# duanyiqun/DiffusionDepth

Hardware: NVIDIA H100
Metric: depth maps/sec @ KITTI 352x1216, Swin-L, 20 DDIM steps (higher is better)
Workload: dtype f32 (fp32-grade products on wgmma: 3-pass fp16 split, fp32 accumulate)

## Files before the change

### diffusiondepth_b200/csrc/conv_halo.cuh

```cuda
#pragma once
#include "conv_common.cuh"

namespace dd {

constexpr int HALO_TH = 16;
constexpr int HALO_TW = 8;

template <int CIN, int COUT, int BK>
struct HaloCfg {
  static_assert(BK == 16 || BK == 32, "bad K chunk");
  static_assert((CIN % BK == 0 || CIN < BK) && CIN % 16 == 0, "bad K chunk");
  static constexpr int KC = (CIN + BK - 1) / BK;
  static constexpr int KSTEPS = (CIN < BK ? CIN : BK) / 16;
  static constexpr int ROW_BYTES = BK * 2;
  static constexpr int STRIP_ROWS = (HALO_TH + 2) * HALO_TW;
  static constexpr int STRIP_BYTES = STRIP_ROWS * ROW_BYTES;
  static constexpr int STRIP_PAD = (STRIP_BYTES + 1023) / 1024 * 1024;
  static constexpr int DX_STRIDE = 2 * STRIP_PAD;
  static constexpr int A_SLOT = 3 * DX_STRIDE;
  static constexpr int A_SLOTS = 2;
  static constexpr int B_TILE = COUT * ROW_BYTES;
  static constexpr int B_TILE_PAD = (B_TILE + 1023) / 1024 * 1024;
  static constexpr int B_SLOT = 2 * B_TILE_PAD;
  static constexpr int NWG = COUT > 128 ? 2 : 1;
  static constexpr int NW = COUT / NWG;
  static constexpr int THREADS = 128 * (1 + NWG);
  static constexpr int CH = NWG > 1 ? 16 : (NW < 32 ? NW : 32);
  static constexpr int LD = CH + 1;
  static constexpr int STAGE_BYTES = NWG * 128 * LD * 4;
  static constexpr int CTRL_BYTES = 1024;
  static constexpr int BUDGET = 227 * 1024 - 1024 - CTRL_BYTES - STAGE_BYTES - A_SLOTS * A_SLOT;
  static constexpr int B_SLOTS_RAW = BUDGET / B_SLOT;
  static constexpr bool B_RESIDENT = (9 * KC * B_SLOT <= 40 * 1024) && (9 * KC <= B_SLOTS_RAW);
  static constexpr int B_SLOTS = B_RESIDENT ? 9 * KC : (B_SLOTS_RAW > 8 ? 8 : B_SLOTS_RAW);
  static_assert(B_SLOTS >= 2, "B ring too small");
  static_assert(NWG == 1 || B_SLOTS >= 3, "256-wide layers: the producer must be able to run two taps ahead");
  static constexpr int SMEM_BYTES = A_SLOTS * A_SLOT + B_SLOTS * B_SLOT + 1024 + CTRL_BYTES + STAGE_BYTES;
  static_assert(SMEM_BYTES <= 232448, "exceeds the 227 KB dynamic shared memory limit");
  static constexpr int A_TX = 6 * STRIP_BYTES;
  static constexpr int B_TX = 2 * B_TILE;
  static constexpr int GROUP_CH = COUT / 4;
  static constexpr int GPW = NW >= GROUP_CH ? NW / GROUP_CH : 1;
  static_assert(NW % GROUP_CH == 0, "a warpgroup's columns cover whole GroupNorm groups");
};

template <int CIN, int COUT, int BK, int EPI>
__global__ void __launch_bounds__((HaloCfg<CIN, COUT, BK>::THREADS), 1)
conv3x3_halo_kernel(const __grid_constant__ CUtensorMap tmA_hi, const __grid_constant__ CUtensorMap tmA_lo,
                    const __grid_constant__ CUtensorMap tmB_hi, const __grid_constant__ CUtensorMap tmB_lo,
                    const ConvArgs p) {
  using C = HaloCfg<CIN, COUT, BK>;
  constexpr int NW = C::NW;
  extern __shared__ uint8_t smem_raw[];
  uint8_t* smem = reinterpret_cast<uint8_t*>((reinterpret_cast<uintptr_t>(smem_raw) + 1023) & ~uintptr_t(1023));
  uint8_t* a_ring = smem;
  uint8_t* b_ring = smem + C::A_SLOTS * C::A_SLOT;
  uint8_t* ctrl = b_ring + C::B_SLOTS * C::B_SLOT;
  uint64_t* a_full = reinterpret_cast<uint64_t*>(ctrl);
  uint64_t* a_empty = a_full + C::A_SLOTS;
  uint64_t* b_full = a_empty + C::A_SLOTS;
  uint64_t* b_empty = b_full + C::B_SLOTS;
  double* red = reinterpret_cast<double*>(b_empty + C::B_SLOTS);
  float* stage = reinterpret_cast<float*>(ctrl + C::CTRL_BYTES);

  const int warp = threadIdx.x >> 5;
  const int lane = threadIdx.x & 31;

  if (threadIdx.x == 0) {
    tma_prefetch_desc(&tmA_hi);
    tma_prefetch_desc(&tmA_lo);
    tma_prefetch_desc(&tmB_hi);
    tma_prefetch_desc(&tmB_lo);
    for (int s = 0; s < C::A_SLOTS; ++s) {
      mbar_init(&a_full[s], 1);
      mbar_init(&a_empty[s], C::NWG);
    }
    for (int s = 0; s < C::B_SLOTS; ++s) {
      mbar_init(&b_full[s], 1);
      mbar_init(&b_empty[s], C::NWG);
    }
    fence_barrier_init();
  }
  __syncthreads();

  if (warp < 4) {
    if constexpr (C::NWG > 1) setmaxnreg_dec<40>();
    if (warp == 0) {
      const bool leader = elect_one();
      int sa = 0;
      uint32_t pa = 0;
      for (int tile = blockIdx.x; tile < p.num_tiles; tile += gridDim.x) {
        const int tx = tile % p.tiles_x, ty = (tile / p.tiles_x) % p.tiles_y, img = tile / (p.tiles_x * p.tiles_y);
        const int x0 = tx * HALO_TW, y0 = ty * HALO_TH;
        for (int kc = 0; kc < C::KC; ++kc) {
          mbar_wait(&a_empty[sa], pa ^ 1);
          uint8_t* s = a_ring + sa * C::A_SLOT;
          if (leader) {
            mbar_arrive_expect_tx(&a_full[sa], C::A_TX);
#pragma unroll
            for (int dx = 0; dx < 3; ++dx) {
              tma_load_4d(s + (2 * dx) * C::STRIP_PAD, &tmA_hi, &a_full[sa], kc * BK, x0 + dx - 1, y0 - 1, img);
              tma_load_4d(s + (2 * dx + 1) * C::STRIP_PAD, &tmA_lo, &a_full[sa], kc * BK, x0 + dx - 1, y0 - 1, img);
            }
          }
          __syncwarp();
          if (++sa == C::A_SLOTS) {
            sa = 0;
            pa ^= 1;
          }
        }
      }
    } else if (warp == 1) {
      const bool leader = elect_one();
      int sb = 0;
      uint32_t pb = 0;
      for (int tile = blockIdx.x; tile < p.num_tiles; tile += gridDim.x) {
        if (C::B_RESIDENT && tile != static_cast<int>(blockIdx.x)) break;
        for (int kc = 0; kc < C::KC; ++kc) {
          for (int tap = 0; tap < 9; ++tap) {
            mbar_wait(&b_empty[sb], pb ^ 1);
            uint8_t* s = b_ring + sb * C::B_SLOT;
            if (leader) {
              mbar_arrive_expect_tx(&b_full[sb], C::B_TX);
              tma_load_3d(s, &tmB_hi, &b_full[sb], kc * BK, 0, tap);
              tma_load_3d(s + C::B_TILE_PAD, &tmB_lo, &b_full[sb], kc * BK, 0, tap);
            }
            __syncwarp();
            if (++sb == C::B_SLOTS) {
              sb = 0;
              pb ^= 1;
            }
          }
        }
      }
    }
  } else {
    if constexpr (C::NWG > 1) setmaxnreg_inc<232>();
    const int wg = (warp >> 2) - 1;
    const int t = threadIdx.x & 127;
    const int q = t >> 5;
    const bool signal = (t == 0);
    float* S = stage + wg * 128 * C::LD;
    const int m = t;
    const int r = m >> 3, c = m & 7;
    const uint32_t b_off = static_cast<uint32_t>(wg * NW);
    int sa = 0, sb = 0, par = 0;
    uint32_t pa = 0, pb = 0;
    float acc[2][NW / 2];

    for (int tile = blockIdx.x; tile < p.num_tiles; tile += gridDim.x) {
      int prev_b = -1, prev_a = -1;
      auto retire_prev = [&]() {
        mbar_arrive_if(&b_empty[prev_b < 0 ? 0 : prev_b], signal && prev_b >= 0);
        mbar_arrive_if(&a_empty[prev_a < 0 ? 0 : prev_a], signal && prev_a >= 0);
        prev_b = prev_a = -1;
      };
      {
        for (int kc = 0; kc < C::KC; ++kc) {
          mbar_wait(&a_full[sa], pa);
          const uint32_t a_base = smem_u32(a_ring + sa * C::A_SLOT);
          for (int tap = 0; tap < 9; ++tap) {
            const int dy = tap / 3, dx = tap % 3;
            mbar_wait(&b_full[sb], C::B_RESIDENT ? 0u : pb);
            const uint32_t sa_hi = a_base + dx * C::DX_STRIDE + dy * HALO_TW * C::ROW_BYTES;
            const uint32_t sa_lo = sa_hi + C::STRIP_PAD;
            const uint32_t sb_hi = smem_u32(b_ring + sb * C::B_SLOT) + b_off * C::ROW_BYTES;
            const uint32_t sb_lo = sb_hi + C::B_TILE_PAD;
            wgmma_fence();
#pragma unroll
            for (int h = 0; h < 2; ++h) {
              const uint32_t ho = static_cast<uint32_t>(h * 64 * C::ROW_BYTES);
#pragma unroll
              for (int k = 0; k < C::KSTEPS; ++k) {
                const uint64_t a_hi = wgmma_desc(sa_hi + ho + k * 32, C::ROW_BYTES);
                const uint64_t a_lo = wgmma_desc(sa_lo + ho + k * 32, C::ROW_BYTES);
                const uint64_t b_hi = wgmma_desc(sb_hi + k * 32, C::ROW_BYTES);
                const uint64_t b_lo = wgmma_desc(sb_lo + k * 32, C::ROW_BYTES);
                wgmma_f16<NW>(acc[h], a_lo, b_hi, (kc | tap | k) != 0 ? 1u : 0u);
                wgmma_f16<NW>(acc[h], a_hi, b_lo, 1u);
                wgmma_f16<NW>(acc[h], a_hi, b_hi, 1u);
              }
            }
            wgmma_commit();
            wgmma_wait<1>();
            retire_prev();
            if (!C::B_RESIDENT) prev_b = sb;
            if (tap == 8) prev_a = sa;
            if (++sb == C::B_SLOTS) {
              sb = 0;
              pb ^= 1;
            }
          }
          if (++sa == C::A_SLOTS) {
            sa = 0;
            pa ^= 1;
          }
        }
      }
      wgmma_wait<0>();
      wgmma_fence_regs(acc[0]);
      wgmma_fence_regs(acc[1]);
      retire_prev();

      const int tx = tile % p.tiles_x, ty = (tile / p.tiles_x) % p.tiles_y, img = tile / (p.tiles_x * p.tiles_y);
      const int x = tx * HALO_TW + c, y = ty * HALO_TH + r;
      const bool valid = (x < p.W) && (y < p.H);
      const size_t pix = (static_cast<size_t>(img) * p.H + y) * p.W + x;
      const uint32_t vmask = __ballot_sync(0xffffffffu, valid);
      const uint32_t row_off = static_cast<uint32_t>(pix * COUT);
      float tk[C::GPW], tsum[C::GPW], tsq[C::GPW];
#pragma unroll
      for (int g = 0; g < C::GPW; ++g) tk[g] = tsum[g] = tsq[g] = 0.f;
      bool overflow = false;
#pragma unroll
      for (int cj = 0; cj < NW / C::CH; ++cj) {
        const int ch0 = wg * NW + cj * C::CH;
        named_bar_sync(2 + wg, 128);
        stage_acc_cols<NW, C::CH, C::LD>(acc[0], S, 0, cj * C::CH / 8);
        stage_acc_cols<NW, C::CH, C::LD>(acc[1], S, 64, cj * C::CH / 8);
        named_bar_sync(2 + wg, 128);
        float v[C::CH];
#pragma unroll
        for (int j = 0; j < C::CH; ++j) v[j] = fmaf(S[m * C::LD + j], p.acc_scale, __ldg(p.bias + ch0 + j));
        if constexpr (EPI == EPI_F32_STATS) {
          if (valid) {
#pragma unroll
            for (int j = 0; j < C::CH; ++j) {
              const int g = (cj * C::CH + j) / C::GROUP_CH;
              if ((cj * C::CH + j) % C::GROUP_CH == 0) tk[g] = v[j];
              const float d = v[j] - tk[g];
              tsum[g] += d;
              tsq[g] = fmaf(d, d, tsq[g]);
            }
          }
        }
        if constexpr (EPI == EPI_F32_STATS || EPI == EPI_F32) {
#pragma unroll
          for (int j = 0; j < C::CH; ++j) S[m * C::LD + j] = v[j];
          __syncwarp();
          if constexpr (C::CH == 32) {
#pragma unroll 8
            for (int rw = 0; rw < 32; ++rw) {
              const uint32_t o = __shfl_sync(0xffffffffu, row_off, rw) + ch0 + lane;
              if ((vmask >> rw) & 1u) p.y32[o] = S[(q * 32 + rw) * C::LD + lane];
            }
          } else {
            constexpr int RPI = 32 / C::CH;
            const int hsel = lane / C::CH, cl = lane % C::CH;
#pragma unroll 8
            for (int i = 0; i < 32 / RPI; ++i) {
              const int rw = RPI * i + hsel;
              const uint32_t o = __shfl_sync(0xffffffffu, row_off, rw) + ch0 + cl;
              if ((vmask >> rw) & 1u) p.y32[o] = S[(q * 32 + rw) * C::LD + cl];
            }
          }
        } else if (valid) {
          {
            __align__(16) __half hi[C::CH];
            __align__(16) __half lo[C::CH];
#pragma unroll
            for (int j = 0; j < C::CH; ++j) {
              const float s = v[j] * p.split_scale;
              overflow |= (fabsf(s) > 60000.f);
              hi[j] = __float2half_rn(s);
              lo[j] = __float2half_rn(s - __half2float(hi[j]));
            }
            uint4* dh = reinterpret_cast<uint4*>(p.out_hi + pix * COUT + ch0);
            uint4* dl = reinterpret_cast<uint4*>(p.out_lo + pix * COUT + ch0);
#pragma unroll
            for (int j = 0; j < C::CH / 8; ++j) {
              dh[j] = reinterpret_cast<const uint4*>(hi)[j];
              dl[j] = reinterpret_cast<const uint4*>(lo)[j];
            }
          }
        }
      }

      if constexpr (EPI == EPI_F32_STATS) {
        const int cw = wg * 4 + q;
#pragma unroll
        for (int k = 0; k < C::GPW; ++k) {
          const double n = valid ? C::GROUP_CH : 0, kk = tk[k], ds = tsum[k];
          double s = fma(n, kk, ds), s2 = fma(n * kk, kk, fma(2.0 * kk, ds, static_cast<double>(tsq[k])));
#pragma unroll
          for (int o = 16; o > 0; o >>= 1) {
            s += __shfl_xor_sync(0xffffffffu, s, o);
            s2 += __shfl_xor_sync(0xffffffffu, s2, o);
          }
          if (lane == 0) {
            red[((par * 4 * C::NWG + cw) * C::GPW + k) * 2 + 0] = s;
            red[((par * 4 * C::NWG + cw) * C::GPW + k) * 2 + 1] = s2;
          }
        }
        named_bar_sync(1, 128 * C::NWG);
        const int e = threadIdx.x - 128;
        if (e < 8) {
          const int g = e >> 1, which = e & 1;
          const int w0 = C::NWG > 1 ? (g / C::GPW) * 4 : 0, k = C::NWG > 1 ? g % C::GPW : g;
          double tt = 0.0;
#pragma unroll
          for (int w = 0; w < 4 * C::NWG; ++w)
            if (C::NWG == 1 || (w >= w0 && w < w0 + 4)) tt += red[((par * 4 * C::NWG + w) * C::GPW + k) * 2 + which];
          p.stats_partial[(static_cast<size_t>(tile) * 4 + g) * 2 + which] = tt;
        }
        par ^= 1;
      }
      if constexpr (EPI == EPI_SPLIT) {
        if (overflow) atomicOr(p.status, 1);
      }
    }
  }
}

}
```

### diffusiondepth_b200/csrc/engine.cu

```cuda
#include <cuda.h>
#include <cuda_runtime.h>
#include <math.h>
#include <stdio.h>
#include <stdlib.h>
#include <string.h>

#include <algorithm>
#include <map>
#include <string>
#include <vector>

#include "../../include/dd_engine.h"
#include "kernels.cuh"
#include "convgen.cuh"
#include "conv_halo.cuh"
#include "pred_fold.cuh"
#include "swin.cuh"
#include "mpvit.cuh"
#include "backward.cuh"
#include "codec_train.cuh"
#include "producer_train.cuh"

namespace {

// ... 65 lines not shown

int encode_map(CUtensorMap* m, const char* what, cuuint32_t rank, const __half* base, const cuuint64_t* dims,
               const cuuint64_t* strides, const cuuint32_t* box, const cuuint32_t* estr, CUtensorMapSwizzle swizzle,
               CUtensorMapL2promotion l2) {
  const CUresult r = g_encode(m, CU_TENSOR_MAP_DATA_TYPE_FLOAT16, rank, const_cast<__half*>(base), dims, strides, box, estr,
                              CU_TENSOR_MAP_INTERLEAVE_NONE, swizzle, l2, CU_TENSOR_MAP_FLOAT_OOB_FILL_NONE);
  if (r != CUDA_SUCCESS)
    return fail(DD_ERR_CUDA, std::string("cuTensorMapEncodeTiled(") + what + ") failed: " + std::to_string((int)r));
  return DD_OK;
}

int make_nhwc_map(CUtensorMap* m, const char* what, const __half* base, int B, int H, int W, int C, int box_c, int box_w,
                  int box_h, CUtensorMapSwizzle swizzle, int stride = 1, int ld = 0) {
  const cuuint64_t L = ld > 0 ? ld : C;
  const cuuint64_t dims[4] = {(cuuint64_t)C, (cuuint64_t)W, (cuuint64_t)H, (cuuint64_t)B};
  const cuuint64_t strides[3] = {L * 2, (cuuint64_t)W * L * 2, (cuuint64_t)H * W * L * 2};
  const cuuint32_t box[4] = {(cuuint32_t)box_c, (cuuint32_t)box_w, (cuuint32_t)box_h, 1};
  const cuuint32_t estr[4] = {1, (cuuint32_t)stride, (cuuint32_t)stride, 1};
  return encode_map(m, what, 4, base, dims, strides, box, estr, swizzle, CU_TENSOR_MAP_L2_PROMOTION_L2_128B);
}
int make_act_map(CUtensorMap* m, const __half* base, int B, int H, int W, int C, int bk, int stride = 1, int ld = 0) {
  return make_nhwc_map(m, "activation", base, B, H, W, C, bk, dd::TILE_W * stride, dd::TILE_H * stride, swizzle_for(bk),
                       stride, ld);
}
int make_patch_map(CUtensorMap* m, const __half* base, int B, int H, int W) {
  const cuuint64_t px = 256 * 2;
  const cuuint64_t dims[5] = {8, (cuuint64_t)H, (cuuint64_t)W, 32, (cuuint64_t)B};
  const cuuint64_t strides[4] = {(cuuint64_t)W * px, px, 16, (cuuint64_t)H * W * px};
  const cuuint32_t box[5] = {8, dd::F5::PH, dd::F5::PW, 2, 1};
  const cuuint32_t estr[5] = {1, 1, 1, 1, 1};
  return encode_map(m, "patch", 5, base, dims, strides, box, estr, CU_TENSOR_MAP_SWIZZLE_NONE,
                    CU_TENSOR_MAP_L2_PROMOTION_L2_128B);
}
int make_weight_map(CUtensorMap* m, const __half* base, int cout, int cin, int taps, int box_k, int rows, int ld = 0) {
  const cuuint64_t L = ld > 0 ? ld : cin;
  const cuuint64_t dims[3] = {(cuuint64_t)cin, (cuuint64_t)cout, (cuuint64_t)taps};
  const cuuint64_t strides[2] = {L * 2, (cuuint64_t)cout * L * 2};
  const cuuint32_t box[3] = {(cuuint32_t)box_k, (cuuint32_t)rows, 1};
  const cuuint32_t estr[3] = {1, 1, 1};
  return encode_map(m, "weight", 3, base, dims, strides, box, estr, swizzle_for(box_k), CU_TENSOR_MAP_L2_PROMOTION_L2_256B);
}

struct ShapeInfo {
  int cin, cout;
};
constexpr ShapeInfo kShapes[5] = {{16, 64}, {64, 256}, {256, 256}, {256, 64}, {64, 16}};
int shape_id(int cin, int cout) {
  for (int i = 0; i < 5; ++i)
    if (kShapes[i].cin == cin && kShapes[i].cout == cout) return i;
  return -1;
}

constexpr int kHaloBK[5] = {16, 32, 32, 32, 32};

template <int CIN, int COUT, int BK, int EPI>
void conv3x3_kernel(bool simt, const dd::SimtArgs& sa, const CUtensorMap* m, const dd::ConvArgs& a, int sm_count,
                    cudaStream_t st) {
  if (simt) {
    constexpr int CO_T = COUT < 64 ? COUT : 64;
    dd::conv3x3_simt_kernel<CIN, COUT, EPI><<<dim3(a.num_tiles, COUT / CO_T), 256, 0, st>>>(sa);
  } else {
    using C = dd::HaloCfg<CIN, COUT, BK>;
    const int grid = a.num_tiles < sm_count ? a.num_tiles : sm_count;
    dd::conv3x3_halo_kernel<CIN, COUT, BK, EPI><<<grid, C::THREADS, C::SMEM_BYTES, st>>>(m[0], m[1], m[2], m[3], a);
  }
}
template <int CIN, int COUT, int BK>
void conv3x3_epi(int epi, bool simt, const dd::SimtArgs& sa, const CUtensorMap* m, const dd::ConvArgs& a, int sm_count,
                 cudaStream_t st) {
  if (epi == dd::EPI_F32_STATS) conv3x3_kernel<CIN, COUT, BK, dd::EPI_F32_STATS>(simt, sa, m, a, sm_count, st);
  else if (epi == dd::EPI_SPLIT) conv3x3_kernel<CIN, COUT, BK, dd::EPI_SPLIT>(simt, sa, m, a, sm_count, st);
  else conv3x3_kernel<CIN, COUT, BK, dd::EPI_F32>(simt, sa, m, a, sm_count, st);
}

int launch_conv3x3(int sid, int epi, bool simt, dd::ConvArgs& a, const __half* in_hi, const __half* in_lo,
                   float in_scale, const float* w_simt, const CUtensorMap& w_hi, const CUtensorMap& w_lo, int sm_count,
                   cudaStream_t st) {
  const int tw = simt ? dd::TILE_W : dd::HALO_TW, th = simt ? dd::TILE_H : dd::HALO_TH;
  a.tiles_x = (a.W + tw - 1) / tw;
  a.tiles_y = (a.H + th - 1) / th;
  a.num_tiles = a.tiles_x * a.tiles_y * a.B;
  CUtensorMap m[4] = {{}, {}, w_hi, w_lo};
  dd::SimtArgs sa{};
  if (simt) {
    sa.in_hi = in_hi;
    sa.in_lo = in_lo;
    sa.in_inv_scale = 1.f / in_scale;
    sa.w = w_simt;
    sa.c = a;
  } else {
    const int cin = kShapes[sid].cin, bk = kHaloBK[sid];
    int rc;
    if ((rc = make_nhwc_map(&m[0], "strip", in_hi, a.B, a.H, a.W, cin, bk, dd::HALO_TW, dd::HALO_TH + 2, swizzle_for(bk))))
      return rc;
    if ((rc = make_nhwc_map(&m[1], "strip", in_lo, a.B, a.H, a.W, cin, bk, dd::HALO_TW, dd::HALO_TH + 2, swizzle_for(bk))))
      return rc;
  }
  switch (sid) {
    case 0: conv3x3_epi<16, 64, kHaloBK[0]>(epi, simt, sa, m, a, sm_count, st); break;
    case 1: conv3x3_epi<64, 256, kHaloBK[1]>(epi, simt, sa, m, a, sm_count, st); break;
    case 2: conv3x3_epi<256, 256, kHaloBK[2]>(epi, simt, sa, m, a, sm_count, st); break;
    case 3: conv3x3_epi<256, 64, kHaloBK[3]>(epi, simt, sa, m, a, sm_count, st); break;
    case 4: conv3x3_epi<64, 16, kHaloBK[4]>(epi, simt, sa, m, a, sm_count, st); break;
    default: return fail(DD_ERR_UNSUPPORTED, "unsupported conv shape");
  }
  return DD_OK;
}

template <int CIN, int COUT, int BK>
cudaError_t configure_halo_all_epi() {
  using C = dd::HaloCfg<CIN, COUT, BK>;
  cudaError_t e;
  if ((e = cudaFuncSetAttribute(dd::conv3x3_halo_kernel<CIN, COUT, BK, dd::EPI_F32_STATS>,
                                cudaFuncAttributeMaxDynamicSharedMemorySize, C::SMEM_BYTES)) != cudaSuccess) return e;
  if ((e = cudaFuncSetAttribute(dd::conv3x3_halo_kernel<CIN, COUT, BK, dd::EPI_SPLIT>,
                                cudaFuncAttributeMaxDynamicSharedMemorySize, C::SMEM_BYTES)) != cudaSuccess) return e;
  return cudaFuncSetAttribute(dd::conv3x3_halo_kernel<CIN, COUT, BK, dd::EPI_F32>,
                              cudaFuncAttributeMaxDynamicSharedMemorySize, C::SMEM_BYTES);
}
template <int MCO, int NCI>
cudaError_t configure_wgm() {
  return cudaFuncSetAttribute(dd::wgrad_wgmma_kernel<MCO, NCI>, cudaFuncAttributeMaxDynamicSharedMemorySize,
                              dd::WgmCfg<MCO, NCI>::SMEM_BYTES);
}
template <int NT>
cudaError_t configure_gen() {
  return cudaFuncSetAttribute(dd::convgen_wgmma_kernel<NT>, cudaFuncAttributeMaxDynamicSharedMemorySize,
                              dd::GenCfg<NT>::SMEM_BYTES);
}
cudaError_t configure_all_kernels() {
  cudaError_t e;
  if ((e = cudaFuncSetAttribute(dd::window_attention_wgmma_kernel, cudaFuncAttributeMaxDynamicSharedMemorySize,
                                dd::WAU_SMEM)) != cudaSuccess) return e;
  if ((e = cudaFuncSetAttribute(dd::decoder_kernel, cudaFuncAttributeMaxDynamicSharedMemorySize, dd::DEC_SMEM)) != cudaSuccess)
    return e;
  if ((e = configure_halo_all_epi<16, 64, 16>()) != cudaSuccess) return e;
  if ((e = configure_halo_all_epi<64, 256, 32>()) != cudaSuccess) return e;
  if ((e = configure_halo_all_epi<256, 256, 32>()) != cudaSuccess) return e;
  if ((e = configure_halo_all_epi<256, 64, 32>()) != cudaSuccess) return e;
  if ((e = configure_halo_all_epi<64, 16, 32>()) != cudaSuccess) return e;
  if ((e = cudaFuncSetAttribute(dd::conv5x5_fold_kernel, cudaFuncAttributeMaxDynamicSharedMemorySize,
                                dd::F5::SMEM_BYTES)) != cudaSuccess) return e;
  if ((e = cudaFuncSetAttribute(dd::ring_fix_kernel, cudaFuncAttributeMaxDynamicSharedMemorySize, dd::RING_SMEM)) !=
      cudaSuccess) return e;
  if ((e = configure_wgm<128, 128>()) != cudaSuccess) return e;
  if ((e = configure_wgm<128, 64>()) != cudaSuccess) return e;
  if ((e = configure_wgm<64, 128>()) != cudaSuccess) return e;
  if ((e = configure_gen<256>()) != cudaSuccess) return e;
  if ((e = configure_gen<192>()) != cudaSuccess) return e;
  if ((e = configure_gen<128>()) != cudaSuccess) return e;
  return configure_gen<64>();
}

struct ConvLayer {
  int sid = -1;
  __half* w_hi = nullptr;
  __half* w_lo = nullptr;
  float* w_simt = nullptr;
  float* bias = nullptr;
  float wscale = 1.f;
  CUtensorMap mh_hi, mh_lo;
};

struct PackStage {
  float amax[16];
  float dec_wt[16 * 16 * 16], dec_bt[16], dec_g[16], dec_be[16], dec_mu[16], dec_var[16], dec_wc[16 * 9], dec_bc[1];
  float enc_w1[144], enc_bn1[4][16], enc_w2[2304], enc_bn2[4][16];
  float wt_f[4 * 4 * 16 * 16], bt_f[16], wc_f[9 * 16], wu[4 * 4 * 16 * 16], bn[3 * 16];
  float f1[144], t1[16], f2[2304], t2[16];
  float e1u[144], e2u[2304], enc_gb[4][16];
  float enc_bn[2][3][16];
};

struct Raw {
  const float* ptr;
  std::vector<int64_t> shape;
};

struct GenLayer {
  int cin = 0, cout = 0, taps = 1, nt = 256, relu = 1, shuffle = 0;
  int stride = 1, add_first = 0;
  __half* w_hi = nullptr;
  __half* w_lo = nullptr;
  float* shift = nullptr;
  float wscale = 1.f;
  CUtensorMap mb_hi, mb_lo;
  bool alt = false;
  CUtensorMap mb_hi_alt, mb_lo_alt;
  float* zero_shift = nullptr;
  int bn = -1;
};

constexpr int kGenSplitIters = 110;
// ... 845 lines not shown
int poll_status(dd_engine* h, cudaStream_t st) {
  CUDA_TRY(cudaMemcpyAsync(h->status_host, h->status, 4, cudaMemcpyDeviceToHost, st));
  CUDA_TRY(cudaStreamSynchronize(st));
  if (*h->status_host & 1)
    return fail(DD_ERR_RANGE, "an activation exceeded the operand split's range (16 |v| > 6e4)");
  return DD_OK;
}

int finish_forward(dd_engine* h, cudaStream_t st) {
  return (h->cfg.flags & DD_FLAG_CHECK_RANGE) ? poll_status(h, st) : DD_OK;
}

void invalidate_pack(dd_engine* h) {
  h->weights_ready = h->packed = false;
  h->ws = nullptr;
  drop_graphs(h);
}

int check_status_word(const int* status, cudaStream_t st, const char* what) {
  int flag = 0;
  CUDA_TRY(cudaMemcpyAsync(&flag, status, 4, cudaMemcpyDeviceToHost, st));
  CUDA_TRY(cudaStreamSynchronize(st));
  if (flag) return fail(DD_ERR_RANGE, std::string("non-finite or out-of-range value in ") + what);
  return DD_OK;
}

const Raw* find(dd_engine* e, const std::string& k) {
  auto it = e->raw.find(k);
  return it == e->raw.end() ? nullptr : &it->second;
}

int dev_alloc(std::vector<void*>& owned, void** p, size_t bytes) {
  cudaError_t err = cudaMalloc(p, bytes);
  if (err != cudaSuccess) return fail(DD_ERR_CUDA, std::string("cudaMalloc: ") + cudaGetErrorString(err));
  owned.push_back(*p);
  return DD_OK;
}
int dev_alloc(dd_engine* e, void** p, size_t bytes) { return dev_alloc(e->owned, p, bytes); }

template <typename T>
int dev_array(dd_engine* e, T** p, size_t elems) {
  return dev_alloc(e->owned, reinterpret_cast<void**>(p), elems * sizeof(T));
}

int alloc_layer(dd_engine* e, ConvLayer& L, int cout, int cin) {
  L.sid = shape_id(cin, cout);
  if (L.sid < 0) return fail(DD_ERR_UNSUPPORTED, "unsupported conv shape");
  const size_t n = static_cast<size_t>(cout) * cin * 9;
  int rc;
  if ((rc = dev_array(e, &L.w_hi, n))) return rc;
  if ((rc = dev_array(e, &L.w_lo, n))) return rc;
  if ((rc = dev_array(e, &L.w_simt, n))) return rc;
  if ((rc = dev_array(e, &L.bias, cout))) return rc;
  if ((rc = make_weight_map(&L.mh_hi, L.w_hi, cout, cin, 9, kHaloBK[L.sid], cout))) return rc;
  return make_weight_map(&L.mh_lo, L.w_lo, cout, cin, 9, kHaloBK[L.sid], cout);
}

constexpr float kProdScale = 16.f;

void bn_fold_host(const float* const* bn, int ch, float* scale, float* shift) {
  for (int c = 0; c < ch; ++c) {
    const double sc = static_cast<double>(bn[0][c]) / sqrt(static_cast<double>(bn[3][c]) + 1e-5);
    scale[c] = static_cast<float>(sc);
    shift[c] = static_cast<float>(static_cast<double>(bn[1][c]) - static_cast<double>(bn[2][c]) * sc);
  }
}
int bn_fold(const float* const* bn, int ch, std::vector<float>& scale, std::vector<float>& shift, cudaStream_t st) {
  std::vector<float> v[4];
  for (int i = 0; i < 4; ++i) {
    v[i].resize(ch);
    CUDA_TRY(cudaMemcpyAsync(v[i].data(), bn[i], ch * 4, cudaMemcpyDeviceToHost, st));
  }
  CUDA_TRY(cudaStreamSynchronize(st));
  scale.resize(ch);
  shift.resize(ch);
  const float* host[4] = {v[0].data(), v[1].data(), v[2].data(), v[3].data()};
  bn_fold_host(host, ch, scale.data(), shift.data());
  return DD_OK;
}
int find_bn(dd_engine* e, const std::string& prefix, const float** bn) {
  const char* parts[4] = {".weight", ".bias", ".running_mean", ".running_var"};
  for (int i = 0; i < 4; ++i) {
    const Raw* r = find(e, prefix + parts[i]);
    if (!r) return fail(DD_ERR_INVALID, "missing weights: " + prefix + parts[i]);
    bn[i] = r->ptr;
  }
  return DD_OK;
}
int copy_param(dd_engine* e, const std::string& key, size_t n, float** out, cudaStream_t st) {
  const Raw* r = find(e, key);
  if (!r) return fail(DD_ERR_INVALID, "missing weights: " + key);
  size_t have = 1;
  for (int64_t d : r->shape) have *= static_cast<size_t>(d);
  if (have != n) return fail(DD_ERR_INVALID, "weight shape mismatch: " + key);
  int rc;
  if ((rc = dev_alloc(e, reinterpret_cast<void**>(out), n * 4))) return rc;
  CUDA_TRY(cudaMemcpyAsync(*out, r->ptr, n * 4, cudaMemcpyDeviceToDevice, st));
  return DD_OK;
}

const char* const kGnKey[4] = {"model.noise_embedding.1", "model.noise_embedding.4", "model.pred.1", "model.pred.4"};
constexpr int kGnCh[4] = {64, 256, 64, 16};
const std::string kDecPrefix = "depth_transform.conv_inv_transform.";
const std::string kEncPrefix = "depth_transform.conv_transform.";
struct CodecKey {
  const char* leaf;
  size_t host_off;
  std::vector<int64_t> shape;
// ... 2292 lines not shown

int dd_poll_status(dd_handle h, void* cuda_stream) {
  if (!h) return fail(DD_ERR_INVALID, "null handle");
  if (!h->status) return DD_OK;
  CUDA_TRY(cudaSetDevice(h->cfg.device));
  return poll_status(h, static_cast<cudaStream_t>(cuda_stream));
}

size_t dd_conv3x3_workspace_bytes(int32_t batch, int32_t cin, int32_t cout, int32_t height, int32_t width) {
  Conv3x3Ws v;
  return conv3x3_layout(nullptr, batch, cin, cout, height, width, v);
}

int dd_conv3x3(dd_handle h, const float* x, const float* w, const float* b, float* y, int32_t batch, int32_t cin,
               int32_t cout, int32_t height, int32_t width, void* workspace, size_t workspace_bytes, void* cuda_stream) {
  if (!h || !x || !w || !b || !y) return fail(DD_ERR_INVALID, "null argument");
  const int sid = shape_id(cin, cout);
  if (sid < 0) return fail(DD_ERR_UNSUPPORTED, "conv shape not on the DiffusionDepth hot path");
  if (workspace_bytes < dd_conv3x3_workspace_bytes(batch, cin, cout, height, width) ||
      (reinterpret_cast<uintptr_t>(workspace) & 1023))
    return fail(DD_ERR_INVALID, "conv workspace too small or misaligned");
  cudaStream_t st = static_cast<cudaStream_t>(cuda_stream);
  CUDA_TRY(cudaSetDevice(h->cfg.device));
  const size_t BP = static_cast<size_t>(batch) * height * width;
  const size_t nw = static_cast<size_t>(cin) * cout * 9;
  Conv3x3Ws v;
  conv3x3_layout(workspace, batch, cin, cout, height, width, v);
  CUDA_TRY(cudaMemsetAsync(v.status, 0, 64, st));
  int rc;
  if ((rc = transpose_in(x, v.xn, batch, cin, height * width, st))) return rc;
  float* amax_dev = reinterpret_cast<float*>(v.status) + 8;
  float sx, sw;
  if ((rc = split_scale_of(v.xn, std::min<size_t>(BP * cin, 1u << 30), amax_dev, st, &sx))) return rc;
  if ((rc = split_scale_of(w, nw, amax_dev, st, &sw))) return rc;
  dd::split_planes_kernel<<<132 * 8, 256, 0, st>>>(v.xn, v.x.hi, v.x.lo, BP * cin / 4, sx, v.status);
  if ((rc = check_launch("split_planes"))) return rc;
  dd::pack_conv_weight_kernel<<<128, 256, 0, st>>>(w, v.w.hi, v.w.lo, v.wsimt, cout, cin, sw);
  if ((rc = check_launch("pack_conv_weight"))) return rc;
  dd::ConvArgs a;
  a.B = batch;
  a.H = height;
  a.W = width;
  a.bias = b;
  a.acc_scale = 1.f / (sx * sw);
  a.y32 = v.yn;
  a.stats_partial = nullptr;
  a.out_hi = nullptr;
  a.out_lo = nullptr;
  a.split_scale = 1.f;
  a.status = v.status;
  const bool simt = (h->cfg.flags & DD_FLAG_SIMT_CONV) != 0;
  CUtensorMap mb_hi{}, mb_lo{};
  if (!simt) {
    if ((rc = make_weight_map(&mb_hi, v.w.hi, cout, cin, 9, kHaloBK[sid], cout))) return rc;
    if ((rc = make_weight_map(&mb_lo, v.w.lo, cout, cin, 9, kHaloBK[sid], cout))) return rc;
  }
  if ((rc = launch_conv3x3(sid, dd::EPI_F32, simt, a, v.x.hi, v.x.lo, sx, v.wsimt, mb_hi, mb_lo, h->sm_count, st)))
    return rc;
  if ((rc = check_launch("conv3x3"))) return rc;
  return transpose_out(v.yn, y, batch, cout, height * width, st);
}

size_t dd_conv3x3_wgrad_workspace_bytes(int32_t batch, int32_t cin, int32_t cout, int32_t height, int32_t width) {
  WgradWs v;
  return wgrad_layout(nullptr, batch, cin, cout, height, width, v);
}

int dd_conv3x3_wgrad(dd_handle h, const float* x, const float* dy, float* dw, float* db, int32_t batch, int32_t cin,
                     int32_t cout, int32_t height, int32_t width, void* workspace, size_t workspace_bytes,
                     void* cuda_stream) {
  if (!h || !x || !dy || !dw || !db) return fail(DD_ERR_INVALID, "null argument");
  if (shape_id(cin, cout) < 0) return fail(DD_ERR_UNSUPPORTED, "conv shape not on the DiffusionDepth hot path");
  if (batch < 1 || height < 1 || width < 1) return fail(DD_ERR_INVALID, "empty geometry");
  if (workspace_bytes < dd_conv3x3_wgrad_workspace_bytes(batch, cin, cout, height, width) ||
      (reinterpret_cast<uintptr_t>(workspace) & 1023))
    return fail(DD_ERR_INVALID, "wgrad workspace too small or misaligned");
  cudaStream_t st = static_cast<cudaStream_t>(cuda_stream);
  CUDA_TRY(cudaSetDevice(h->cfg.device));
  const int P = height * width;
  const size_t BP = static_cast<size_t>(batch) * P;
  WgradWs v;
  wgrad_layout(workspace, batch, cin, cout, height, width, v);
  float* scratch = reinterpret_cast<float*>(v.status) + 8;
  CUDA_TRY(cudaMemsetAsync(v.status, 0, 64, st));
  int rc;
  if ((rc = transpose_in(x, v.xn, batch, cin, P, st))) return rc;
  if ((rc = transpose_in(dy, v.dyn, batch, cout, P, st))) return rc;
  float sx;
  if ((rc = split_scale_of(v.xn, BP * cin, scratch, st, &sx))) return rc;
  dd::split_planes_kernel<<<132 * 8, 256, 0, st>>>(v.xn, v.x.hi, v.x.lo, BP * cin / 4, sx, v.status);
  if ((rc = launched(h, "split_planes"))) return rc;
  if ((rc = run_colsum(h, cout, v.dyn, nullptr, batch, P, v.col_part, nullptr, db, st))) return rc;
  const WgradBufs bufs{v.dy, scratch + 1, scratch + 2, v.status, v.partial};
  if ((rc = run_wgrad(h, batch, height, width, cout, cin, v.dyn, nullptr, v.x.hi, v.x.lo, sx, dw, true, bufs, st)))
    return rc;
  return check_status_word(v.status, st, "x or dy");
}

int dd_gen_layer(dd_handle h, const dd_gen_layer_desc* d, const float* x0, const float* x1, const float* w,
                 const float* bias, const float* const* bn, const float* add32, float* y32, void* out_hi, void* out_lo,
                 int32_t* launch_out, void* cuda_stream) {
  if (!h || !d || !x0 || !w || (d->c1 > 0 && !x1)) return fail(DD_ERR_INVALID, "null argument");
  if (!y32 && !(out_hi && out_lo)) return fail(DD_ERR_INVALID, "no output");
  const bool gemm = d->tokens > 0, xp = d->transposed != 0;
  const int c0 = d->c0, c1 = d->c1, cout = d->cout;
  const int cin = d->cin > 0 ? d->cin : c0 + c1;
  if ((d->taps != 1 && d->taps != 9) || (d->stride != 1 && d->stride != 2) || d->act < 0 || d->act > 3 || c0 < 8 ||
      c1 < 0 || c0 % 8 || c1 % 8 || cout < 8 || cin > c0 + c1 || (cin < c0 + c1 && c1 > 0))
// ... 234 lines not shown
                      float* y32, float* mean_rstd, float* out, void* cuda_stream) {
  if (!h || !d || !x || !w || !b || !gamma || !beta) return fail(DD_ERR_INVALID, "null argument");
  const int B = d->batch, cin = d->cin, cout = d->cout, H = d->height, W = d->width, mode = d->mode;
  const int sid = shape_id(cin, cout);
  if (sid < 0 || (cin == 256 && cout == 256)) return fail(DD_ERR_UNSUPPORTED, "not a GroupNorm'd conv of the DDIM loop");
  if (B < 1 || H < 1 || W < 1 || mode < 0 || mode > 3) return fail(DD_ERR_INVALID, "bad conv / GroupNorm descriptor");
  if ((mode == 0 && cout != 64) || ((mode == 1 || mode == 2) && cout != 256) || (mode == 3 && cout != 16))
    return fail(DD_ERR_UNSUPPORTED, "the loop applies that mode to another conv shape");
  if ((mode == 1 || mode == 2) && (!cond || !temb)) return fail(DD_ERR_INVALID, "null condition or time embedding");
  if (mode == 2 && (d->cond_h < 1 || d->cond_w < 1 || (d->up_qpb != 4 && d->up_qpb != 1)))
    return fail(DD_ERR_INVALID, "bad up-add geometry");
  cudaStream_t st = static_cast<cudaStream_t>(cuda_stream);
  CUDA_TRY(cudaSetDevice(h->cfg.device));
  const int P = H * W;
  const size_t BP = static_cast<size_t>(B) * P;
  const size_t nw = static_cast<size_t>(cin) * cout * 9;
  const int ch = mode == 2 ? d->cond_h : H, cw = mode == 2 ? d->cond_w : W;
  StandaloneCall call(h);
  int rc;
  if ((rc = call.begin(st))) return rc;
  float* scratch = reinterpret_cast<float*>(call.status) + 8;
  const bool simt = (h->cfg.flags & DD_FLAG_SIMT_CONV) != 0;
  const int tiles_img = simt ? ((W + dd::TILE_W - 1) / dd::TILE_W) * ((H + dd::TILE_H - 1) / dd::TILE_H)
                             : ((W + dd::HALO_TW - 1) / dd::HALO_TW) * ((H + dd::HALO_TH - 1) / dd::HALO_TH);
  float *xn, *yn, *wsimt, *mr, *cn = nullptr, *xl = nullptr, *eps = nullptr;
  double* partial;
  Planes xs, wp, o;
  if ((rc = call.alloc(&xn, BP * cin)) || (rc = call.alloc(&xs.hi, BP * cin)) || (rc = call.alloc(&xs.lo, BP * cin)) ||
      (rc = call.alloc(&yn, BP * cout)) || (rc = call.alloc(&wp.hi, nw)) || (rc = call.alloc(&wp.lo, nw)) ||
      (rc = call.alloc(&wsimt, nw)) || (rc = call.alloc(&partial, static_cast<size_t>(B) * tiles_img * 8)) ||
      (rc = call.alloc(&mr, static_cast<size_t>(B) * 8)) || (rc = call.alloc(&o.hi, BP * cout)) ||
      (rc = call.alloc(&o.lo, BP * cout)))
    return rc;
  if ((rc = transpose_in(x, xn, B, cin, P, st))) return rc;
  const float sx = cin == 16 ? kXScale : kActScale;
  float sw;
  if ((rc = split_scale_of(w, nw, scratch, st, &sw))) return rc;
  if ((rc = split_planes(h, xn, xs.hi, xs.lo, BP * cin, sx, st))) return rc;
  dd::pack_conv_weight_kernel<<<128, 256, 0, st>>>(w, wp.hi, wp.lo, wsimt, cout, cin, sw);
  if ((rc = check_launch("pack_conv_weight"))) return rc;
  dd::ConvArgs a;
  a.B = B;
  a.H = H;
  a.W = W;
  a.bias = b;
  a.acc_scale = 1.f / (sx * sw);
  a.y32 = yn;
  a.stats_partial = partial;
  a.out_hi = a.out_lo = nullptr;
  a.split_scale = 1.f;
  a.status = call.status;
  CUtensorMap mb_hi{}, mb_lo{};
  if (!simt) {
    if ((rc = make_weight_map(&mb_hi, wp.hi, cout, cin, 9, kHaloBK[sid], cout))) return rc;
    if ((rc = make_weight_map(&mb_lo, wp.lo, cout, cin, 9, kHaloBK[sid], cout))) return rc;
  }
  if ((rc = launch_conv3x3(sid, dd::EPI_F32_STATS, simt, a, xs.hi, xs.lo, sx, wsimt, mb_hi, mb_lo, h->sm_count, st)))
    return rc;
  if ((rc = check_launch("conv3x3"))) return rc;
  dd::gn_finalize_kernel<<<B * 4, 256, 0, st>>>(partial, a.tiles_x * a.tiles_y, nullptr, 0,
                                                 1.0 / (static_cast<double>(P) * (cout / 4)), 1e-5f, mr);
  if ((rc = check_launch("gn_finalize"))) return rc;
  if (mode == 3) {
    dd::FinalArgs f;
    f.y = yn;
    f.mean_rstd = mr;
    f.gamma = gamma;
    f.beta = beta;
    f.x = nullptr;
    f.x_hi = o.hi;
    f.x_lo = o.lo;
    f.eps_out = nullptr;
    f.cx = d->c_x;
    f.ce = d->c_eps;
    f.scale = kXScale;
    f.P = P;
    f.status = call.status;
    if (latent) {
      if ((rc = call.alloc(&xl, BP * 16)) || (rc = transpose_in(latent, xl, B, 16, P, st))) return rc;
      f.x = xl;
    } else {
      if ((rc = call.alloc(&eps, BP * 16))) return rc;
      f.eps_out = eps;
    }
    launch_final(f, B, st);
    if ((rc = check_launch("gn_relu_ddim"))) return rc;
  } else {
    dd::ApplyArgs g;
    g.y = yn;
    g.mean_rstd = mr;
    g.gamma = gamma;
    g.beta = beta;
    g.cond = nullptr;
    g.temb = temb;
    g.temb_bstride = 256;
    g.H = H;
    g.W = W;
    g.ch = ch;
    g.cw = cw;
    g.ry = H > 1 ? static_cast<float>(ch - 1) / static_cast<float>(H - 1) : 0.f;
    g.rx = W > 1 ? static_cast<float>(cw - 1) / static_cast<float>(W - 1) : 0.f;
    g.out_hi = o.hi;
    g.out_lo = o.lo;
    g.scale = kActScale;
    g.status = call.status;
    if (mode != 0) {
      const size_t nc = static_cast<size_t>(B) * ch * cw * 256;
      if ((rc = call.alloc(&cn, nc)) || (rc = transpose_in(cond, cn, B, 256, ch * cw, st))) return rc;
// ... 56 lines not shown
```

Measured before the change: 28.44.

## Run multiple halo-conv CTAs per SM and split wide output columns across units

The halo 3x3 conv kernel gains two per-shape settings. SPLIT divides the output channels into independent work units, each loading its own weight row slice. CTAS sets how many CTAs share an SM: shared memory, register reallocation and the A-ring depth are derived from it, and the launch grid is sized from the occupancy API. This aims to raise SM occupancy and overlap between CTAs for the small-channel layers, and to balance work for the 64->256 layer. In exchange, each CTA gets a single A slot in some configs with a full wgmma drain per K chunk, split layers stream their weights rather than keeping them resident, and the per-CTA register budget shrinks.

Result: faster. 28.74, median of 6 (+1.0%).

```diff
diff --git a/diffusiondepth_b200/csrc/conv_halo.cuh b/diffusiondepth_b200/csrc/conv_halo.cuh
--- a/diffusiondepth_b200/csrc/conv_halo.cuh
+++ b/diffusiondepth_b200/csrc/conv_halo.cuh
@@ -6,10 +6,11 @@
 constexpr int HALO_TH = 16;
 constexpr int HALO_TW = 8;
 
-template <int CIN, int COUT, int BK>
+template <int CIN, int COUT, int BK, int SPLIT = 1, int CTAS = 1>
 struct HaloCfg {
   static_assert(BK == 16 || BK == 32, "bad K chunk");
   static_assert((CIN % BK == 0 || CIN < BK) && CIN % 16 == 0, "bad K chunk");
+  static_assert(CTAS >= 1 && CTAS <= 3, "one to three CTAs per SM");
   static constexpr int KC = (CIN + BK - 1) / BK;
   static constexpr int KSTEPS = (CIN < BK ? CIN : BK) / 16;
   static constexpr int ROW_BYTES = BK * 2;
@@ -18,39 +19,49 @@
   static constexpr int STRIP_PAD = (STRIP_BYTES + 1023) / 1024 * 1024;
   static constexpr int DX_STRIDE = 2 * STRIP_PAD;
   static constexpr int A_SLOT = 3 * DX_STRIDE;
-  static constexpr int A_SLOTS = 2;
-  static constexpr int B_TILE = COUT * ROW_BYTES;
+  static constexpr int NCOL = COUT / SPLIT;
+  static_assert(COUT % SPLIT == 0, "bad column split");
+  static constexpr int B_TILE = NCOL * ROW_BYTES;
   static constexpr int B_TILE_PAD = (B_TILE + 1023) / 1024 * 1024;
   static constexpr int B_SLOT = 2 * B_TILE_PAD;
-  static constexpr int NWG = COUT > 128 ? 2 : 1;
-  static constexpr int NW = COUT / NWG;
+  static constexpr int NWG = NCOL > 128 ? 2 : 1;
+  static constexpr int NW = NCOL / NWG;
   static constexpr int THREADS = 128 * (1 + NWG);
-  static constexpr int CH = NWG > 1 ? 16 : (NW < 32 ? NW : 32);
+  static constexpr bool REALLOC = NWG > 1 || CTAS > 1;
+  static constexpr int REGS_CAP = 65536 / (THREADS * CTAS) / 8 * 8;
+  static constexpr int PRODUCER_REGS = 40;
+  static constexpr int CONSUMER_REGS = (REGS_CAP * (1 + NWG) - PRODUCER_REGS) / NWG / 8 * 8;
+  static constexpr int CH = CTAS > 2 ? 8 : (NWG > 1 || CTAS > 1) ? 16 : (NW < 32 ? NW : 32);
   static constexpr int LD = CH + 1;
   static constexpr int STAGE_BYTES = NWG * 128 * LD * 4;
   static constexpr int CTRL_BYTES = 1024;
-  static constexpr int BUDGET = 227 * 1024 - 1024 - CTRL_BYTES - STAGE_BYTES - A_SLOTS * A_SLOT;
+  static constexpr int SMEM_LIMIT = CTAS == 1 ? 227 * 1024 : 228 * 1024 / CTAS - 1024;
+  static constexpr int FIXED_BYTES = 1024 + CTRL_BYTES + STAGE_BYTES;
+  static constexpr int A_SLOTS = SMEM_LIMIT - FIXED_BYTES - 2 * A_SLOT >= 3 * B_SLOT ? 2 : 1;
+  static constexpr int BUDGET = SMEM_LIMIT - FIXED_BYTES - A_SLOTS * A_SLOT;
   static constexpr int B_SLOTS_RAW = BUDGET / B_SLOT;
-  static constexpr bool B_RESIDENT = (9 * KC * B_SLOT <= 40 * 1024) && (9 * KC <= B_SLOTS_RAW);
+  static constexpr bool B_RESIDENT = SPLIT == 1 && (9 * KC * B_SLOT <= 40 * 1024) && (9 * KC <= B_SLOTS_RAW);
   static constexpr int B_SLOTS = B_RESIDENT ? 9 * KC : (B_SLOTS_RAW > 8 ? 8 : B_SLOTS_RAW);
   static_assert(B_SLOTS >= 2, "B ring too small");
-  static_assert(NWG == 1 || B_SLOTS >= 3, "256-wide layers: the producer must be able to run two taps ahead");
-  static constexpr int SMEM_BYTES = A_SLOTS * A_SLOT + B_SLOTS * B_SLOT + 1024 + CTRL_BYTES + STAGE_BYTES;
-  static_assert(SMEM_BYTES <= 232448, "exceeds the 227 KB dynamic shared memory limit");
+  static_assert(B_RESIDENT || B_SLOTS >= 3, "streamed weights: the producer must be able to run two taps ahead");
+  static constexpr int SMEM_BYTES = A_SLOTS * A_SLOT + B_SLOTS * B_SLOT + FIXED_BYTES;
+  static_assert(SMEM_BYTES <= SMEM_LIMIT, "exceeds the per-CTA dynamic shared memory limit");
   static constexpr int A_TX = 6 * STRIP_BYTES;
   static constexpr int B_TX = 2 * B_TILE;
   static constexpr int GROUP_CH = COUT / 4;
   static constexpr int GPW = NW >= GROUP_CH ? NW / GROUP_CH : 1;
+  static constexpr int UNIT_GROUPS = NCOL / GROUP_CH;
   static_assert(NW % GROUP_CH == 0, "a warpgroup's columns cover whole GroupNorm groups");
 };
 
-template <int CIN, int COUT, int BK, int EPI>
-__global__ void __launch_bounds__((HaloCfg<CIN, COUT, BK>::THREADS), 1)
+template <int CIN, int COUT, int BK, int SPLIT, int CTAS, int EPI>
+__global__ void __launch_bounds__((HaloCfg<CIN, COUT, BK, SPLIT, CTAS>::THREADS), CTAS)
 conv3x3_halo_kernel(const __grid_constant__ CUtensorMap tmA_hi, const __grid_constant__ CUtensorMap tmA_lo,
                     const __grid_constant__ CUtensorMap tmB_hi, const __grid_constant__ CUtensorMap tmB_lo,
                     const ConvArgs p) {
-  using C = HaloCfg<CIN, COUT, BK>;
+  using C = HaloCfg<CIN, COUT, BK, SPLIT, CTAS>;
   constexpr int NW = C::NW;
+  const int units = p.num_tiles * SPLIT;
   extern __shared__ uint8_t smem_raw[];
   uint8_t* smem = reinterpret_cast<uint8_t*>((reinterpret_cast<uintptr_t>(smem_raw) + 1023) & ~uintptr_t(1023));
   uint8_t* a_ring = smem;
@@ -84,12 +95,13 @@
   __syncthreads();
 
   if (warp < 4) {
-    if constexpr (C::NWG > 1) setmaxnreg_dec<40>();
+    if constexpr (C::REALLOC) setmaxnreg_dec<C::PRODUCER_REGS>();
     if (warp == 0) {
       const bool leader = elect_one();
       int sa = 0;
       uint32_t pa = 0;
-      for (int tile = blockIdx.x; tile < p.num_tiles; tile += gridDim.x) {
+      for (int u = blockIdx.x; u < units; u += gridDim.x) {
+        const int tile = u / SPLIT;
         const int tx = tile % p.tiles_x, ty = (tile / p.tiles_x) % p.tiles_y, img = tile / (p.tiles_x * p.tiles_y);
         const int x0 = tx * HALO_TW, y0 = ty * HALO_TH;
         for (int kc = 0; kc < C::KC; ++kc) {
@@ -114,16 +126,17 @@
       const bool leader = elect_one();
       int sb = 0;
       uint32_t pb = 0;
-      for (int tile = blockIdx.x; tile < p.num_tiles; tile += gridDim.x) {
-        if (C::B_RESIDENT && tile != static_cast<int>(blockIdx.x)) break;
+      for (int u = blockIdx.x; u < units; u += gridDim.x) {
+        if (C::B_RESIDENT && u != static_cast<int>(blockIdx.x)) break;
+        const int row0 = (u % SPLIT) * C::NCOL;
         for (int kc = 0; kc < C::KC; ++kc) {
           for (int tap = 0; tap < 9; ++tap) {
             mbar_wait(&b_empty[sb], pb ^ 1);
             uint8_t* s = b_ring + sb * C::B_SLOT;
             if (leader) {
               mbar_arrive_expect_tx(&b_full[sb], C::B_TX);
-              tma_load_3d(s, &tmB_hi, &b_full[sb], kc * BK, 0, tap);
-              tma_load_3d(s + C::B_TILE_PAD, &tmB_lo, &b_full[sb], kc * BK, 0, tap);
+              tma_load_3d(s, &tmB_hi, &b_full[sb], kc * BK, row0, tap);
+              tma_load_3d(s + C::B_TILE_PAD, &tmB_lo, &b_full[sb], kc * BK, row0, tap);
             }
             __syncwarp();
             if (++sb == C::B_SLOTS) {
@@ -135,7 +148,7 @@
       }
     }
   } else {
-    if constexpr (C::NWG > 1) setmaxnreg_inc<232>();
+    if constexpr (C::REALLOC) setmaxnreg_inc<C::CONSUMER_REGS>();
     const int wg = (warp >> 2) - 1;
     const int t = threadIdx.x & 127;
     const int q = t >> 5;
@@ -148,7 +161,8 @@
     uint32_t pa = 0, pb = 0;
     float acc[2][NW / 2];
 
-    for (int tile = blockIdx.x; tile < p.num_tiles; tile += gridDim.x) {
+    for (int u = blockIdx.x; u < units; u += gridDim.x) {
+      const int tile = u / SPLIT, col0 = (u % SPLIT) * C::NCOL;
       int prev_b = -1, prev_a = -1;
       auto retire_prev = [&]() {
         mbar_arrive_if(&b_empty[prev_b < 0 ? 0 : prev_b], signal && prev_b >= 0);
@@ -191,6 +205,10 @@
               pb ^= 1;
             }
           }
+          if constexpr (C::A_SLOTS == 1) {
+            wgmma_wait<0>();
+            retire_prev();
+          }
           if (++sa == C::A_SLOTS) {
             sa = 0;
             pa ^= 1;
@@ -214,7 +232,7 @@
       bool overflow = false;
 #pragma unroll
       for (int cj = 0; cj < NW / C::CH; ++cj) {
-        const int ch0 = wg * NW + cj * C::CH;
+        const int ch0 = col0 + wg * NW + cj * C::CH;
         named_bar_sync(2 + wg, 128);
         stage_acc_cols<NW, C::CH, C::LD>(acc[0], S, 0, cj * C::CH / 8);
         stage_acc_cols<NW, C::CH, C::LD>(acc[1], S, 64, cj * C::CH / 8);
@@ -294,14 +312,14 @@
         }
         named_bar_sync(1, 128 * C::NWG);
         const int e = threadIdx.x - 128;
-        if (e < 8) {
+        if (e < 2 * C::UNIT_GROUPS) {
           const int g = e >> 1, which = e & 1;
-          const int w0 = C::NWG > 1 ? (g / C::GPW) * 4 : 0, k = C::NWG > 1 ? g % C::GPW : g;
+          const int w0 = (g / C::GPW) * 4, k = g % C::GPW;
           double tt = 0.0;
 #pragma unroll
-          for (int w = 0; w < 4 * C::NWG; ++w)
-            if (C::NWG == 1 || (w >= w0 && w < w0 + 4)) tt += red[((par * 4 * C::NWG + w) * C::GPW + k) * 2 + which];
-          p.stats_partial[(static_cast<size_t>(tile) * 4 + g) * 2 + which] = tt;
+          for (int w = w0; w < w0 + 4; ++w) tt += red[((par * 4 * C::NWG + w) * C::GPW + k) * 2 + which];
+          const int gt = col0 / C::GROUP_CH + g;
+          p.stats_partial[(static_cast<size_t>(tile) * 4 + gt) * 2 + which] = tt;
         }
         par ^= 1;
       }
diff --git a/diffusiondepth_b200/csrc/engine.cu b/diffusiondepth_b200/csrc/engine.cu
--- a/diffusiondepth_b200/csrc/engine.cu
+++ b/diffusiondepth_b200/csrc/engine.cu
@@ -141,25 +141,42 @@
 }
 
 constexpr int kHaloBK[5] = {16, 32, 32, 32, 32};
-
-template <int CIN, int COUT, int BK, int EPI>
+constexpr int kHaloSplit[5] = {1, 2, 1, 1, 1};
+constexpr int kHaloCtas[5] = {2, 2, 1, 1, 3};
+
+template <int SID>
+using HaloCfgOf = dd::HaloCfg<kShapes[SID].cin, kShapes[SID].cout, kHaloBK[SID], kHaloSplit[SID], kHaloCtas[SID]>;
+template <int SID, int EPI>
+constexpr auto halo_kernel =
+    dd::conv3x3_halo_kernel<kShapes[SID].cin, kShapes[SID].cout, kHaloBK[SID], kHaloSplit[SID], kHaloCtas[SID], EPI>;
+template <int SID, int EPI>
+int halo_blocks_per_sm = 1;
+
+int make_halo_weight_map(CUtensorMap* m, const __half* w, int sid) {
+  const int cin = kShapes[sid].cin, cout = kShapes[sid].cout;
+  return make_weight_map(m, w, cout, cin, 9, kHaloBK[sid], cout / kHaloSplit[sid]);
+}
+
+template <int SID, int EPI>
 void conv3x3_kernel(bool simt, const dd::SimtArgs& sa, const CUtensorMap* m, const dd::ConvArgs& a, int sm_count,
                     cudaStream_t st) {
+  constexpr int CIN = kShapes[SID].cin, COUT = kShapes[SID].cout;
   if (simt) {
     constexpr int CO_T = COUT < 64 ? COUT : 64;
     dd::conv3x3_simt_kernel<CIN, COUT, EPI><<<dim3(a.num_tiles, COUT / CO_T), 256, 0, st>>>(sa);
   } else {
-    using C = dd::HaloCfg<CIN, COUT, BK>;
-    const int grid = a.num_tiles < sm_count ? a.num_tiles : sm_count;
-    dd::conv3x3_halo_kernel<CIN, COUT, BK, EPI><<<grid, C::THREADS, C::SMEM_BYTES, st>>>(m[0], m[1], m[2], m[3], a);
-  }
-}
-template <int CIN, int COUT, int BK>
+    using C = HaloCfgOf<SID>;
+    const int units = a.num_tiles * kHaloSplit[SID], slots = halo_blocks_per_sm<SID, EPI> * sm_count;
+    const int grid = units < slots ? units : slots;
+    halo_kernel<SID, EPI><<<grid, C::THREADS, C::SMEM_BYTES, st>>>(m[0], m[1], m[2], m[3], a);
+  }
+}
+template <int SID>
 void conv3x3_epi(int epi, bool simt, const dd::SimtArgs& sa, const CUtensorMap* m, const dd::ConvArgs& a, int sm_count,
                  cudaStream_t st) {
-  if (epi == dd::EPI_F32_STATS) conv3x3_kernel<CIN, COUT, BK, dd::EPI_F32_STATS>(simt, sa, m, a, sm_count, st);
-  else if (epi == dd::EPI_SPLIT) conv3x3_kernel<CIN, COUT, BK, dd::EPI_SPLIT>(simt, sa, m, a, sm_count, st);
-  else conv3x3_kernel<CIN, COUT, BK, dd::EPI_F32>(simt, sa, m, a, sm_count, st);
+  if (epi == dd::EPI_F32_STATS) conv3x3_kernel<SID, dd::EPI_F32_STATS>(simt, sa, m, a, sm_count, st);
+  else if (epi == dd::EPI_SPLIT) conv3x3_kernel<SID, dd::EPI_SPLIT>(simt, sa, m, a, sm_count, st);
+  else conv3x3_kernel<SID, dd::EPI_F32>(simt, sa, m, a, sm_count, st);
 }
 
 int launch_conv3x3(int sid, int epi, bool simt, dd::ConvArgs& a, const __half* in_hi, const __half* in_lo,
@@ -186,26 +203,37 @@
       return rc;
   }
   switch (sid) {
-    case 0: conv3x3_epi<16, 64, kHaloBK[0]>(epi, simt, sa, m, a, sm_count, st); break;
-    case 1: conv3x3_epi<64, 256, kHaloBK[1]>(epi, simt, sa, m, a, sm_count, st); break;
-    case 2: conv3x3_epi<256, 256, kHaloBK[2]>(epi, simt, sa, m, a, sm_count, st); break;
-    case 3: conv3x3_epi<256, 64, kHaloBK[3]>(epi, simt, sa, m, a, sm_count, st); break;
-    case 4: conv3x3_epi<64, 16, kHaloBK[4]>(epi, simt, sa, m, a, sm_count, st); break;
+    case 0: conv3x3_epi<0>(epi, simt, sa, m, a, sm_count, st); break;
+    case 1: conv3x3_epi<1>(epi, simt, sa, m, a, sm_count, st); break;
+    case 2: conv3x3_epi<2>(epi, simt, sa, m, a, sm_count, st); break;
+    case 3: conv3x3_epi<3>(epi, simt, sa, m, a, sm_count, st); break;
+    case 4: conv3x3_epi<4>(epi, simt, sa, m, a, sm_count, st); break;
     default: return fail(DD_ERR_UNSUPPORTED, "unsupported conv shape");
   }
   return DD_OK;
 }
 
-template <int CIN, int COUT, int BK>
+template <int SID, int EPI>
+cudaError_t configure_halo() {
+  using C = HaloCfgOf<SID>;
+  cudaError_t e;
+  if ((e = cudaFuncSetAttribute(halo_kernel<SID, EPI>, cudaFuncAttributeMaxDynamicSharedMemorySize, C::SMEM_BYTES)) !=
+      cudaSuccess) return e;
+  if ((e = cudaFuncSetAttribute(halo_kernel<SID, EPI>, cudaFuncAttributePreferredSharedMemoryCarveout,
+                                cudaSharedmemCarveoutMaxShared)) != cudaSuccess) return e;
+  int n = 0;
+  if ((e = cudaOccupancyMaxActiveBlocksPerMultiprocessor(&n, halo_kernel<SID, EPI>, C::THREADS, C::SMEM_BYTES)) !=
+      cudaSuccess) return e;
+  if (n < 1) return cudaErrorLaunchOutOfResources;
+  halo_blocks_per_sm<SID, EPI> = n;
+  return cudaSuccess;
+}
+template <int SID>
 cudaError_t configure_halo_all_epi() {
-  using C = dd::HaloCfg<CIN, COUT, BK>;
   cudaError_t e;
-  if ((e = cudaFuncSetAttribute(dd::conv3x3_halo_kernel<CIN, COUT, BK, dd::EPI_F32_STATS>,
-                                cudaFuncAttributeMaxDynamicSharedMemorySize, C::SMEM_BYTES)) != cudaSuccess) return e;
-  if ((e = cudaFuncSetAttribute(dd::conv3x3_halo_kernel<CIN, COUT, BK, dd::EPI_SPLIT>,
-                                cudaFuncAttributeMaxDynamicSharedMemorySize, C::SMEM_BYTES)) != cudaSuccess) return e;
-  return cudaFuncSetAttribute(dd::conv3x3_halo_kernel<CIN, COUT, BK, dd::EPI_F32>,
-                              cudaFuncAttributeMaxDynamicSharedMemorySize, C::SMEM_BYTES);
+  if ((e = configure_halo<SID, dd::EPI_F32_STATS>()) != cudaSuccess) return e;
+  if ((e = configure_halo<SID, dd::EPI_SPLIT>()) != cudaSuccess) return e;
+  return configure_halo<SID, dd::EPI_F32>();
 }
 template <int MCO, int NCI>
 cudaError_t configure_wgm() {
@@ -223,11 +251,11 @@
                                 dd::WAU_SMEM)) != cudaSuccess) return e;
   if ((e = cudaFuncSetAttribute(dd::decoder_kernel, cudaFuncAttributeMaxDynamicSharedMemorySize, dd::DEC_SMEM)) != cudaSuccess)
     return e;
-  if ((e = configure_halo_all_epi<16, 64, 16>()) != cudaSuccess) return e;
-  if ((e = configure_halo_all_epi<64, 256, 32>()) != cudaSuccess) return e;
-  if ((e = configure_halo_all_epi<256, 256, 32>()) != cudaSuccess) return e;
-  if ((e = configure_halo_all_epi<256, 64, 32>()) != cudaSuccess) return e;
-  if ((e = configure_halo_all_epi<64, 16, 32>()) != cudaSuccess) return e;
+  if ((e = configure_halo_all_epi<0>()) != cudaSuccess) return e;
+  if ((e = configure_halo_all_epi<1>()) != cudaSuccess) return e;
+  if ((e = configure_halo_all_epi<2>()) != cudaSuccess) return e;
+  if ((e = configure_halo_all_epi<3>()) != cudaSuccess) return e;
+  if ((e = configure_halo_all_epi<4>()) != cudaSuccess) return e;
   if ((e = cudaFuncSetAttribute(dd::conv5x5_fold_kernel, cudaFuncAttributeMaxDynamicSharedMemorySize,
                                 dd::F5::SMEM_BYTES)) != cudaSuccess) return e;
   if ((e = cudaFuncSetAttribute(dd::ring_fix_kernel, cudaFuncAttributeMaxDynamicSharedMemorySize, dd::RING_SMEM)) !=
@@ -1179,8 +1207,8 @@
   if ((rc = dev_array(e, &L.w_lo, n))) return rc;
   if ((rc = dev_array(e, &L.w_simt, n))) return rc;
   if ((rc = dev_array(e, &L.bias, cout))) return rc;
-  if ((rc = make_weight_map(&L.mh_hi, L.w_hi, cout, cin, 9, kHaloBK[L.sid], cout))) return rc;
-  return make_weight_map(&L.mh_lo, L.w_lo, cout, cin, 9, kHaloBK[L.sid], cout);
+  if ((rc = make_halo_weight_map(&L.mh_hi, L.w_hi, L.sid))) return rc;
+  return make_halo_weight_map(&L.mh_lo, L.w_lo, L.sid);
 }
 
 constexpr float kProdScale = 16.f;
@@ -3579,8 +3607,8 @@
   const bool simt = (h->cfg.flags & DD_FLAG_SIMT_CONV) != 0;
   CUtensorMap mb_hi{}, mb_lo{};
   if (!simt) {
-    if ((rc = make_weight_map(&mb_hi, v.w.hi, cout, cin, 9, kHaloBK[sid], cout))) return rc;
-    if ((rc = make_weight_map(&mb_lo, v.w.lo, cout, cin, 9, kHaloBK[sid], cout))) return rc;
+    if ((rc = make_halo_weight_map(&mb_hi, v.w.hi, sid))) return rc;
+    if ((rc = make_halo_weight_map(&mb_lo, v.w.lo, sid))) return rc;
   }
   if ((rc = launch_conv3x3(sid, dd::EPI_F32, simt, a, v.x.hi, v.x.lo, sx, v.wsimt, mb_hi, mb_lo, h->sm_count, st)))
     return rc;
@@ -3921,8 +3949,8 @@
   a.status = call.status;
   CUtensorMap mb_hi{}, mb_lo{};
   if (!simt) {
-    if ((rc = make_weight_map(&mb_hi, wp.hi, cout, cin, 9, kHaloBK[sid], cout))) return rc;
-    if ((rc = make_weight_map(&mb_lo, wp.lo, cout, cin, 9, kHaloBK[sid], cout))) return rc;
+    if ((rc = make_halo_weight_map(&mb_hi, wp.hi, sid))) return rc;
+    if ((rc = make_halo_weight_map(&mb_lo, wp.lo, sid))) return rc;
   }
   if ((rc = launch_conv3x3(sid, dd::EPI_F32_STATS, simt, a, xs.hi, xs.lo, sx, wsimt, mb_hi, mb_lo, h->sm_count, st)))
     return rc;
```
